# AuroraEchos/Sound-Event-Localization-and-Detection

Measured on AMD Instinct MI355X. Metric: train-step samples/sec (8ch x 128mel x 512T), higher is better.
Workload: dtype f32; 1 GPU; c3: DQSELD-TCN-S1-PHI_8ch train step, F=128 T=512 (U=L=192, SURVEY F3), batch 32/GPU, random-init weights; global_batch=32, parallelism=dp1, step_mode=graph (auto: probe 9.50 ms recorded / 10.73 ms eager per step), deterministic=True

## Files before the change

include/seld_hip.h:

```cpp
#ifndef SELD_HIP_H
#define SELD_HIP_H

#include <stddef.h>
#include <stdint.h>

#ifdef __cplusplus
extern "C" {
#endif

#define SELD_OK            0
#define SELD_EINVAL       -1
#define SELD_EWORKSPACE   -2
#define SELD_ELAUNCH      -3
#define SELD_EUNSUPPORTED -4

int         seld_abi_version(void);
const char* seld_build_arch(void);
int         seld_last_hip_error(void);
int         seld_env_reload(void);
int         seld_tuning_build(void);

typedef struct seld_conv_desc {
    int32_t algebra;
    int32_t ndim;
    int32_t N, Cin, Cout;
    int32_t in[2];
    int32_t k[2];
    int32_t stride[2];
    int32_t pad[2];
    int32_t dil[2];
    int32_t groups;
} seld_conv_desc;

#define SELD_EPI_NONE        0
// ... 210 lines not shown

int seld_bn_act_fwd(const float* x, int32_t N, int32_t C, int32_t S, const float* mean, const float* invstd,
                    const float* gamma, const float* beta, int32_t act, float* y, void* stream);

int seld_bn_act_bwd_reduce(const float* dy, const float* x, const float* y, int32_t N, int32_t C, int32_t S,
                           const float* mean, const float* invstd, const float* gamma, const float* beta,
                           int32_t act, float* dgamma_dbeta , void* stream);
int seld_bn_act_bwd_apply(const float* dy, const float* x, const float* y, int32_t N, int32_t C, int32_t S,
                          const float* mean, const float* invstd, const float* gamma, const float* beta,
                          int32_t act, const float* dgamma_dbeta, int32_t train, float* dx, void* stream);

int seld_bn_act_bwd_fused(const float* dy, const float* x, const float* y, int32_t N, int32_t C, int32_t S,
                          const float* mean, const float* invstd, const float* gamma, int32_t act,
                          float* dgamma_dbeta, const float* dy2, float* dx, void* stream);

int seld_gate_fwd(const float* yf, const float* yg, int32_t N, int32_t C, int32_t S,
                  const float* mean_f, const float* invstd_f, const float* gamma_f, const float* beta_f,
                  const float* mean_g, const float* invstd_g, const float* gamma_g, const float* beta_g,
                  const float* mask, float* y, void* stream);
int seld_gate_bwd_reduce(const float* dy, const float* yf, const float* yg, int32_t N, int32_t C, int32_t S,
                         const float* mean_f, const float* invstd_f, const float* gamma_f, const float* beta_f,
                         const float* mean_g, const float* invstd_g, const float* gamma_g, const float* beta_g,
                         const float* mask, float* red, void* stream);
int seld_gate_bwd_apply(const float* dy, const float* yf, const float* yg, int32_t N, int32_t C, int32_t S,
                        const float* mean_f, const float* invstd_f, const float* gamma_f, const float* beta_f,
                        const float* mean_g, const float* invstd_g, const float* gamma_g, const float* beta_g,
                        const float* mask, const float* red, int32_t train, float* dyf, float* dyg, void* stream);

int seld_hcq_first_pool(const seld_conv_desc* desc, const float* x, const float* wpack, const float* bias,
                        const float* gamma, int32_t want_stats, float* y, float* stats, float* pool_raw, uint8_t* idx,
// ... 10 lines not shown
size_t seld_first_stage_bwd_workspace(const seld_conv_desc* desc);
int seld_first_stage_bwd(const seld_conv_desc* desc, const float* x, const float* dout, const float* out, const float* raw,
                         const uint8_t* idx, const float* mean, const float* invstd, const float* gamma, const float* beta,
                         const float* bias, const double* gram, const float* wg, float* dgamma, float* dbeta,
                         float* const dw[8], float drop_p, void* workspace, size_t workspace_bytes, void* stream);

int seld_bn_pool_finish(const float* raw, int32_t N, int32_t C, int32_t S , const float* mean,
                        const float* invstd, const float* gamma, const float* beta, float* pooled, float p, uint64_t seed,
                        uint64_t offset, const uint64_t* state, float* out, void* stream);

int seld_gate_bwd_fused(const float* dy, const float* yf, const float* yg, int32_t N, int32_t C, int32_t S,
                        const float* mean_f, const float* invstd_f, const float* gamma_f, const float* beta_f,
                        const float* mean_g, const float* invstd_g, const float* gamma_g, const float* beta_g,
                        const float* mask, float* red, float* dyf, float* dyg, void* stream);

size_t seld_hcq_pack_floats(const seld_conv_desc* desc, int32_t mode, int32_t npair);
int seld_hcq_pack(const seld_conv_desc* desc, int32_t mode, int32_t npair, const float* const wA[8],
                  const float* const wB[8], float* wpack, void* stream);
int seld_hcq_conv(const seld_conv_desc* desc, int32_t mode, int32_t npair, const float* x, const float* x2,
                  const float* wpack, float* const y[2], const float* const bias[2], const int32_t epilogue[2],
                  const float* const addend[2], float* const stats[2], void* stream);
int seld_hcq_kernel_label(const seld_conv_desc* desc, int32_t mode, int32_t npair, char* buf, int32_t buflen);
size_t seld_hcq_pack_entry_bytes(void);
int seld_hcq_pack_entry(const seld_conv_desc* desc, int32_t mode, int32_t npair, const float* const wA[8],
                        const float* const wB[8], float* wpack, void* entry_host);
int seld_hcq_pack_table(const void* table_dev, int32_t nentries, int64_t max_floats, void* stream);
int seld_hcq_pack_flat(const void* table_dev, const int32_t* starts_dev, int32_t nentries, int32_t total_blocks,
                       void* stream);

int seld_hcq_wgrad_supported(const seld_conv_desc* desc, int32_t npair);
// ... 132 lines not shown
```

sound-event-localization-and-detection_amd/csrc/abi.hip:

```cpp
#include <mutex>
#include <stdio.h>
#include <stdlib.h>
#include "common.h"
#include "env.h"

namespace seld {
thread_local int g_last_hip_error = 0;

static SeldEnv g_env;
static bool g_env_loaded = false;
static std::mutex g_env_mutex;

static bool flag(const char* name) { const char* e = getenv(name); return e && *e; }
static long long bounded(const char* name, long long lo, long long hi, long long dflt) {
    const char* e = getenv(name);
    if (!e || !*e) return dflt;
    char* end = nullptr;
    const long long v = strtoll(e, &end, 10);
    return (end == e || v < lo || v > hi) ? dflt : v;
}

static void load_env_locked() {
    SeldEnv e;
    if (const char* c = getenv("SELD_CONV_CFG")) {
// ... 3 lines not shown
    e.conv_novec = flag("SELD_CONV_NOVEC");
    e.conv_nofast = flag("SELD_CONV_NOFAST");
    e.conv_no_smallk = flag("SELD_CONV_NO_SMALLK");
    e.no_fwd_pair = flag("SELD_NO_FWD_PAIR");
    e.conv_pair = flag("SELD_CONV_PAIR");
    e.conv_no_hcq = flag("SELD_CONV_NO_HCQ");
    e.hcq_wgrad_dq = flag("SELD_HCQ_WGRAD_DQ");
    e.stft_radix2 = flag("SELD_STFT_RADIX2");
    e.hcq_no_first = flag("SELD_HCQ_NO_FIRST");
    e.hcq_no_pool = flag("SELD_HCQ_NO_POOL");
    e.hcq_wgrad_row = flag("SELD_HCQ_WGRAD_ROW");
    e.deterministic = flag("SELD_DETERMINISTIC");
    e.wgrad_norow = flag("SELD_WGRAD_NOROW");
    e.wgrad_slow = flag("SELD_WGRAD_SLOW");
    e.mha_no_mfma = flag("SELD_MHA_NO_MFMA");
    e.wgrad_cfg = (int)bounded("SELD_WGRAD_CFG", 0, 5, -1);
    e.wgrad_wgs = bounded("SELD_WGRAD_WGS", 1, 1 << 20, 0);
    e.smallk_wgs = bounded("SELD_SMALLK_WGS", 1, 1 << 20, 0);
#ifdef SELD_TUNING
    e.vec_dbg = (int)bounded("SELD_VEC_DBG", 0, 63, 0);
    e.wgrad_dbg = (int)bounded("SELD_WGRAD_DBG", 0, 3, 0);
    e.smallk_dbg = (int)bounded("SELD_SMALLK_DBG", 0, 1023, 0);
    e.smallk_nw = bounded("SELD_SMALLK_NW", 4, 8, 4) == 8 ? 8 : 4;
#endif
    g_env = e;
    g_env_loaded = true;
}

const SeldEnv& env() {
    if (!g_env_loaded) {
// ... 5 lines not shown
}

extern "C" int seld_env_reload(void) {
    std::lock_guard<std::mutex> lk(seld::g_env_mutex);
    seld::load_env_locked();
    return SELD_OK;
}
extern "C" int seld_tuning_build(void) {
#ifdef SELD_TUNING
    return 1;
#else
    return 0;
#endif
}

extern "C" int seld_abi_version(void) { return 2; }
extern "C" const char* seld_build_arch(void) { return "gfx950"; }
extern "C" int seld_last_hip_error(void) { return seld::g_last_hip_error; }
```

sound-event-localization-and-detection_amd/csrc/env.h:

```cpp
#pragma once

namespace seld {

struct SeldEnv {
    int conv_cfg_ct = 0, conv_cfg_pt = 0;
    bool conv_novec = false, conv_nofast = false, conv_no_smallk = false, no_fwd_pair = false, conv_pair = false;
    bool hcq_wgrad_dq = false;
    bool conv_no_hcq = false;
    bool hcq_wgrad_row = false;
    bool hcq_no_pool = false;
    bool stft_radix2 = false;
    bool hcq_no_first = false;
    bool deterministic = false;
    bool wgrad_norow = false, wgrad_slow = false, mha_no_mfma = false;
    int wgrad_cfg = -1;
    long long wgrad_wgs = 0, smallk_wgs = 0;
    int vec_dbg = 0, wgrad_dbg = 0, smallk_dbg = 0, smallk_nw = 4;
};

const SeldEnv& env();

}
```

sound-event-localization-and-detection_amd/csrc/nn_ops.hip:

```cpp
#include "common.h"
#include "env.h"

namespace seld {

__device__ __forceinline__ float act_apply(float z, int act) {
    switch (act) {
        case SELD_ACT_RELU: return z > 0.f ? z : 0.f;
        case SELD_ACT_TANH: return tanhf(z);
        case SELD_ACT_SIGMOID: return 1.0f / (1.0f + expf(-z));
        default: return z;
    }
}
__device__ __forceinline__ float act_grad_from_y(float y, int act) {
    switch (act) {
        case SELD_ACT_RELU: return y > 0.f ? 1.f : 0.f;
        case SELD_ACT_TANH: return 1.f - y * y;
        case SELD_ACT_SIGMOID: return y * (1.f - y);
        default: return 1.f;
    }
}

constexpr int RED_CHUNK = 8192;

template <typename F>
// ... 384 lines not shown
            for (int e = 0; e < 4; ++e) {
                const float t = gate_tanh(ff[e] * af + bf);
                const float sg = gate_sig(gg[e] * ag + bg);
                const float d = dd[e] * mk;
                const float dzf = d * sg * (1.f - t * t);
                const float dzg = d * t * sg * (1.f - sg);
                of[e] = af * (dzf - kf1 - (ff[e] - muf) * isf * kf2);
                og[e] = ag * (dzg - kg1 - (gg[e] - mug) * isg * kg2);
            }
            *reinterpret_cast<float4*>(dyf + base + s) = make_float4(of[0], of[1], of[2], of[3]);
            *reinterpret_cast<float4*>(dyg + base + s) = make_float4(og[0], og[1], og[2], og[3]);
        }
    }
}

constexpr int CH_THREADS = 512;

template <int NV>
__device__ __forceinline__ void channel_block_sum(float (&v)[NV]) {
    __shared__ float part[NV][CH_THREADS / 64];
    const int wave = threadIdx.x >> 6, lane = threadIdx.x & 63;
#pragma unroll
    for (int k = 0; k < NV; ++k) {
        const float s = wave_sum(v[k]);
        if (lane == 0) part[k][wave] = s;
    }
    __syncthreads();
#pragma unroll
    for (int k = 0; k < NV; ++k) {
        float t = 0.f;
#pragma unroll
        for (int w = 0; w < CH_THREADS / 64; ++w) t += part[k][w];
        v[k] = t;
    }
}

__device__ __forceinline__ float4 ld4(const float* p) { return *reinterpret_cast<const float4*>(p); }

template <int PER>
__global__ __launch_bounds__(CH_THREADS) void bn_act_bwd_channel_kernel(
    const float* __restrict__ dy, const float* __restrict__ x, const float* __restrict__ y, int N, int C, int S,
    const float* __restrict__ mean, const float* __restrict__ invstd, const float* __restrict__ gamma, int act,
    float* __restrict__ red, const float* __restrict__ dy2, float* __restrict__ dx, float inv_count) {
    const int c = blockIdx.x;
    const int S4 = S >> 2, G = N * S4;
    const float mu = mean[c], is = invstd[c], a = gamma[c] * is;
    float4 dz[PER], xh[PER];
    float v[2] = {0.f, 0.f};
    float4 ds_[PER], xs_[PER], ys_[PER];
#pragma unroll
    for (int k = 0; k < PER; ++k) {
        const int g = min((int)threadIdx.x + k * CH_THREADS, G - 1);
        const int n = g / S4, s4 = g - n * S4;
        const size_t o = ((size_t)n * C + c) * S + (size_t)s4 * 4;
        ds_[k] = ld4(dy + o); xs_[k] = ld4(x + o); ys_[k] = ld4(y + o);
        if (dy2) {
            const float4 e = ld4(dy2 + o);
            ds_[k].x += e.x; ds_[k].y += e.y; ds_[k].z += e.z; ds_[k].w += e.w;
        }
    }
    __builtin_amdgcn_sched_barrier(0);
// ... 24 lines not shown
        const int g = (int)threadIdx.x + k * CH_THREADS;
        if (g < G) {
            const int n = g / S4, s4 = g - n * S4;
            const size_t o = ((size_t)n * C + c) * S + (size_t)s4 * 4;
            float4 r = make_float4(a * (dz[k].x - k1 - xh[k].x * k2), a * (dz[k].y - k1 - xh[k].y * k2),
                                   a * (dz[k].z - k1 - xh[k].z * k2), a * (dz[k].w - k1 - xh[k].w * k2));
            *reinterpret_cast<float4*>(dx + o) = r;
        }
    }
}

template <int PER>
__global__ __launch_bounds__(CH_THREADS) void gate_bwd_channel_kernel(
    const float* __restrict__ dy, const float* __restrict__ yf, const float* __restrict__ yg, int N, int C, int S,
    GateBN bn, const float* __restrict__ mask, float* __restrict__ red, float* __restrict__ dyf,
    float* __restrict__ dyg, float inv_count) {
    const int c = blockIdx.x;
    const int S4 = S >> 2, G = N * S4;
    const float muf = bn.mean_f[c], isf = bn.invstd_f[c], af = bn.gamma_f[c] * isf, bf = bn.beta_f[c] - muf * af;
    const float mug = bn.mean_g[c], isg = bn.invstd_g[c], ag = bn.gamma_g[c] * isg, bg = bn.beta_g[c] - mug * ag;
    float dzf[PER][4], dzg[PER][4], fh[PER][4], gh[PER][4];
    float v[4] = {0.f, 0.f, 0.f, 0.f};
    float4 d4s[PER], f4s[PER], g4s[PER];
    float mks[PER];
#pragma unroll
    for (int k = 0; k < PER; ++k) {
        const int g = min((int)threadIdx.x + k * CH_THREADS, G - 1);
        const int n = g / S4, s4 = g - n * S4;
        const size_t o = ((size_t)n * C + c) * S + (size_t)s4 * 4;
        d4s[k] = ld4(dy + o); f4s[k] = ld4(yf + o); g4s[k] = ld4(yg + o);
        mks[k] = mask ? mask[n * C + c] : 1.0f;
    }
    __builtin_amdgcn_sched_barrier(0);
#pragma unroll
    for (int k = 0; k < PER; ++k) {
// ... 370 lines not shown
    return check_launch();
}

extern "C" int seld_bn_act_bwd_apply(const float* dy, const float* x, const float* y, int32_t N, int32_t C, int32_t S,
                                     const float* mean, const float* invstd, const float* gamma, const float* beta,
                                     int32_t act, const float* red, int32_t train, float* dx, void* stream) {
    (void)beta;
    if (!dy || !x || !y || !dx || (train && !red)) return SELD_EINVAL;
    const long long total = (long long)N * C * S;
    const float inv_count = 1.0f / (float)((long long)N * S);
    hipLaunchKernelGGL(bn_act_bwd_apply_kernel, dim3(grid_for(total / 4 + 1)), dim3(256), 0, ST(stream), dy, x, y, total,
                       C, S, mean, invstd, gamma, act, red, inv_count, train, dx);
    return check_launch();
}

extern "C" int seld_bn_act_bwd_fused(const float* dy, const float* x, const float* y, int32_t N, int32_t C, int32_t S,
                                     const float* mean, const float* invstd, const float* gamma, int32_t act,
                                     float* red, const float* dy2, float* dx, void* stream) {
    if (!dy || !x || !y || !red || !mean || !invstd || !gamma || N <= 0 || C <= 0 || S <= 0) return SELD_EINVAL;
    const long long G = (long long)N * S / 4;
    if ((S & 3) || G > 16LL * CH_THREADS) return SELD_EUNSUPPORTED;
    const float inv_count = 1.0f / (float)((long long)N * S);
    const int per = (int)((G + CH_THREADS - 1) / CH_THREADS);
#define SELD_BN_CH(P)                                                                                                   \
    hipLaunchKernelGGL(bn_act_bwd_channel_kernel<P>, dim3(C), dim3(CH_THREADS), 0, ST(stream), dy, x, y, N, C, S, mean,  \
                       invstd, gamma, act, red, dy2, dx, inv_count)
    if (per <= 1) SELD_BN_CH(1);
    else if (per <= 2) SELD_BN_CH(2);
    else if (per <= 4) SELD_BN_CH(4);
    else if (per <= 8) SELD_BN_CH(8);
    else SELD_BN_CH(16);
#undef SELD_BN_CH
    return check_launch();
}

static GateBN mk_gate(const float* mean_f, const float* invstd_f, const float* gamma_f, const float* beta_f,
                      const float* mean_g, const float* invstd_g, const float* gamma_g, const float* beta_g) {
    GateBN b{mean_f, invstd_f, gamma_f, beta_f, mean_g, invstd_g, gamma_g, beta_g};
    return b;
}

extern "C" int seld_gate_fwd(const float* yf, const float* yg, int32_t N, int32_t C, int32_t S, const float* mean_f,
                             const float* invstd_f, const float* gamma_f, const float* beta_f, const float* mean_g,
                             const float* invstd_g, const float* gamma_g, const float* beta_g, const float* mask,
                             float* y, void* stream) {
    if (!yf || !yg || !y) return SELD_EINVAL;
    const long long total = (long long)N * C * S;
    if (S % 4 == 0 && (long long)N * C < (1LL << 31))
// ... 28 lines not shown
                                   void* stream) {
    if (!dy || !yf || !yg || !dyf || !dyg || (train && !red)) return SELD_EINVAL;
    const long long total = (long long)N * C * S;
    const float inv_count = 1.0f / (float)((long long)N * S);
    if (S % 4 == 0 && (long long)N * C < (1LL << 31))
        hipLaunchKernelGGL(gate_bwd_apply_row_kernel, dim3(row_grid((long long)N * C)), dim3(256), 0, ST(stream), dy, yf, yg,
                           N * C, C, S, mk_gate(mean_f, invstd_f, gamma_f, beta_f, mean_g, invstd_g, gamma_g, beta_g), mask, red,
                           inv_count, train, dyf, dyg);
    else
        hipLaunchKernelGGL(gate_bwd_apply_kernel, dim3(grid_for(total / 4 + 1)), dim3(256), 0, ST(stream), dy, yf, yg, total,
                           C, S, mk_gate(mean_f, invstd_f, gamma_f, beta_f, mean_g, invstd_g, gamma_g, beta_g), mask, red,
                           inv_count, train, dyf, dyg);
    return check_launch();
}

extern "C" int seld_gate_bwd_fused(const float* dy, const float* yf, const float* yg, int32_t N, int32_t C, int32_t S,
                                   const float* mean_f, const float* invstd_f, const float* gamma_f, const float* beta_f,
                                   const float* mean_g, const float* invstd_g, const float* gamma_g, const float* beta_g,
                                   const float* mask, float* red, float* dyf, float* dyg, void* stream) {
    if (!dy || !yf || !yg || !red || !dyf || !dyg || N <= 0 || C <= 0 || S <= 0) return SELD_EINVAL;
    const long long G = (long long)N * S / 4;
    if ((S & 3) || G > 8LL * CH_THREADS) return SELD_EUNSUPPORTED;
    const float inv_count = 1.0f / (float)((long long)N * S);
    const int per = (int)((G + CH_THREADS - 1) / CH_THREADS);
    const GateBN bn = mk_gate(mean_f, invstd_f, gamma_f, beta_f, mean_g, invstd_g, gamma_g, beta_g);
#define SELD_GATE_CH(P)                                                                                                 \
    hipLaunchKernelGGL(gate_bwd_channel_kernel<P>, dim3(C), dim3(CH_THREADS), 0, ST(stream), dy, yf, yg, N, C, S, bn,    \
                       mask, red, dyf, dyg, inv_count)
    if (per <= 1) SELD_GATE_CH(1);
    else if (per <= 2) SELD_GATE_CH(2);
    else if (per <= 4) SELD_GATE_CH(4);
    else SELD_GATE_CH(8);
#undef SELD_GATE_CH
    return check_launch();
}

extern "C" int seld_act_fwd(const float* x, int64_t n, int32_t act, float* y, void* stream) {
    if (!x || !y || n < 0) return SELD_EINVAL;
    if (n == 0) return SELD_OK;
    hipLaunchKernelGGL(act_fwd_kernel, dim3(grid_for(n)), dim3(256), 0, ST(stream), x, (long long)n, act, y);
    return check_launch();
}
extern "C" int seld_act_bwd(const float* dy, const float* y, int64_t n, int32_t act, float* dx, void* stream) {
    if (!dy || !y || !dx || n < 0) return SELD_EINVAL;
    if (n == 0) return SELD_OK;
    hipLaunchKernelGGL(act_bwd_kernel, dim3(grid_for(n)), dim3(256), 0, ST(stream), dy, y, (long long)n, act, dx);
    return check_launch();
}
// ... 104 lines not shown
```

sound-event-localization-and-detection_amd/hip_ops/norm_act.py:

```python
import os

import torch

from .. import _lib as L
from ._core import _req


def _ncs(x):
    N, C = x.shape[0], x.shape[1]
    S = 1
    for d in x.shape[2:]:
        S *= d
    return N, C, S


STATS_REPLICAS = 64


_stats_pool = {}


def new_stats(C, device):
    free = _stats_pool.get((C, device, torch.cuda.current_stream(device).cuda_stream))
    if free:
        return free.pop()
    t = torch.zeros(STATS_REPLICAS * 2 * C, device=device, dtype=torch.float32)
    t._seld_pooled = True
    return t


def channel_stats(x, out=None):
    N, C, S = _ncs(x)
    stats = out if out is not None else new_stats(C, x.device)
    L.check(L.lib().seld_channel_stats(L.ptr(x), N, C, S, L.ptr(stats), L.current_stream()), "seld_channel_stats")
    return stats


def bn_prepare(x, running_mean, running_var, training, momentum, eps, stats=None, num_batches_tracked=None):
    N, C, S = _ncs(x)
    mean = torch.empty(C, device=x.device, dtype=torch.float32)
    invstd = torch.empty(C, device=x.device, dtype=torch.float32)
    if training:
        if stats is None:
# ... 84 lines not shown
    w._seld_base_param = param
    return w


def axpy_(dst_first, src, n):
    L.check(L.lib().seld_accumulate(L.ptr(dst_first), L.ptr(src), n, L.current_stream()), "seld_accumulate")


def _one_pass_ok(N, S, limit):
    return S % 4 == 0 and N * S <= limit and not os.environ.get("SELD_BN_TWO_PASS")


class BnActFn(torch.autograd.Function):

    @staticmethod
    def forward(ctx, x, gamma, beta, running_mean, running_var, training, momentum, eps, act, stats, nbt, twin):
        x = _req(x, "x")
        N, C, S = _ncs(x)
        mean, invstd = bn_prepare(x, running_mean, running_var, training, momentum, eps, stats, nbt)
        y = torch.empty_like(x)
        L.check(L.lib().seld_bn_act_fwd(L.ptr(x), N, C, S, L.ptr(mean), L.ptr(invstd), L.ptr(gamma), L.ptr(beta),
                                        act, L.ptr(y), L.current_stream()), "seld_bn_act_fwd")
        ctx.training, ctx.act = training, act
        ctx.bn_params = (gamma, beta)
        ctx.save_for_backward(x, y, mean, invstd)
        ctx.twin = twin
        if twin:
            ctx.set_materialize_grads(False)
            return y, y.view_as(y)
        return y

    @staticmethod
    def backward(ctx, dy, dy2=None):
        x, y, mean, invstd = ctx.saved_tensors
        gamma, beta = ctx.bn_params
        if dy is None:
            dy, dy2 = dy2, None
        if dy is None:
            return (None,) * 12
        dy = _req(dy, "dy")
        dy2 = _req(dy2, "dy2") if dy2 is not None else None
        none = (None,) * 9
        N, C, S = _ncs(x)
        slot, clean = _claim_grad_slots((gamma, beta))
        st = L.current_stream()
        if ctx.training and _one_pass_ok(N, S, 32768):
            red = slot if slot is not None else torch.zeros(2 * C, device=x.device, dtype=torch.float32)
            dx = torch.empty_like(x) if ctx.needs_input_grad[0] else None
            L.check(L.lib().seld_bn_act_bwd_fused(L.ptr(dy), L.ptr(x), L.ptr(y), N, C, S, L.ptr(mean), L.ptr(invstd),
                                                  L.ptr(gamma), ctx.act, L.ptr(red), L.ptr(dy2), L.ptr(dx), st),
                    "seld_bn_act_bwd_fused")
            if slot is not None:
                return (dx, None, None) + none
            return (dx, red[:C], red[C:]) + none
        if dy2 is not None:
            dy = dy + dy2
        red = slot if clean else torch.zeros(2 * C, device=x.device, dtype=torch.float32)
        L.check(L.lib().seld_bn_act_bwd_reduce(L.ptr(dy), L.ptr(x), L.ptr(y), N, C, S, L.ptr(mean), L.ptr(invstd),
                                               L.ptr(gamma), L.ptr(beta), ctx.act, L.ptr(red), st),
                "seld_bn_act_bwd_reduce")
        dx = None
        if ctx.needs_input_grad[0]:
            dx = torch.empty_like(x)
            L.check(L.lib().seld_bn_act_bwd_apply(L.ptr(dy), L.ptr(x), L.ptr(y), N, C, S, L.ptr(mean), L.ptr(invstd),
                                                  L.ptr(gamma), L.ptr(beta), ctx.act, L.ptr(red), int(ctx.training),
                                                  L.ptr(dx), st), "seld_bn_act_bwd_apply")
        if slot is not None:
            if not clean:
                axpy_(slot, red, 2 * C)
            return (dx, None, None) + none
        return (dx, red[:C], red[C:]) + none


def bn_act(x, bn, act, stats=None, twin=False):
    return BnActFn.apply(x, bn.weight, bn.bias, bn.running_mean, bn.running_var, bn.training,
                         bn.momentum if bn.momentum is not None else 0.1, bn.eps, act, stats, _nbt(bn), twin)


class GateFn(torch.autograd.Function):

    @staticmethod
    def forward(ctx, yf, yg, gf, bf, rmf, rvf, gg, bg, rmg, rvg, training, momentum, eps, mask, nbt_f, nbt_g,
                stats_f=None, stats_g=None):
        yf, yg = _req(yf, "yf"), _req(yg, "yg")
        N, C, S = _ncs(yf)
        if (training and stats_f is not None and stats_g is not None and getattr(stats_f, "_seld_pooled", False)
                and getattr(stats_g, "_seld_pooled", False)):
            mf, isf, mg, isg = (torch.empty(C, device=yf.device, dtype=torch.float32) for _ in range(4))
            L.check(L.lib().seld_bn_finalize2_ex(L.ptr(stats_f), L.ptr(stats_g), C, N * S, eps, momentum, L.ptr(mf),
                                                 L.ptr(isf), L.ptr(rmf), L.ptr(rvf), L.ptr(nbt_f), L.ptr(mg),
                                                 L.ptr(isg), L.ptr(rmg), L.ptr(rvg), L.ptr(nbt_g), 1,
                                                 L.current_stream()), "seld_bn_finalize2_ex")
            key = (C, yf.device, torch.cuda.current_stream(yf.device).cuda_stream)
            _stats_pool.setdefault(key, []).extend((stats_f, stats_g))
        else:
            mf, isf = bn_prepare(yf, rmf, rvf, training, momentum, eps, stats_f, nbt_f)
            mg, isg = bn_prepare(yg, rmg, rvg, training, momentum, eps, stats_g, nbt_g)
        y = torch.empty_like(yf)
        L.check(L.lib().seld_gate_fwd(L.ptr(yf), L.ptr(yg), N, C, S, L.ptr(mf), L.ptr(isf), L.ptr(gf), L.ptr(bf),
                                      L.ptr(mg), L.ptr(isg), L.ptr(gg), L.ptr(bg), L.ptr(mask), L.ptr(y),
                                      L.current_stream()), "seld_gate_fwd")
        ctx.training = training
        ctx.has_mask = mask is not None
        ctx.bn_params = (gf, bf, gg, bg)
        ctx.save_for_backward(yf, yg, mf, isf, mg, isg, *([mask] if mask is not None else []))
        return y

    @staticmethod
    def backward(ctx, dy):
        yf, yg, mf, isf, mg, isg, *rest = ctx.saved_tensors
        gf, bf, gg, bg = ctx.bn_params
        mask = rest[0] if ctx.has_mask else None
        dy = _req(dy, "dy")
        N, C, S = _ncs(yf)
        slot, clean = _claim_grad_slots((gf, bf, gg, bg))
        st = L.current_stream()
        if ctx.training and _one_pass_ok(N, S, 16384):
            red = slot if slot is not None else torch.zeros(4 * C, device=yf.device, dtype=torch.float32)
            dyf, dyg = torch.empty_like(yf), torch.empty_like(yg)
            L.check(L.lib().seld_gate_bwd_fused(L.ptr(dy), L.ptr(yf), L.ptr(yg), N, C, S, L.ptr(mf), L.ptr(isf),
                                                L.ptr(gf), L.ptr(bf), L.ptr(mg), L.ptr(isg), L.ptr(gg), L.ptr(bg),
                                                L.ptr(mask), L.ptr(red), L.ptr(dyf), L.ptr(dyg), st),
                    "seld_gate_bwd_fused")
            if slot is not None:
                return (dyf, dyg) + (None,) * 16
            return (dyf, dyg, red[:C], red[C:2 * C], None, None, red[2 * C:3 * C], red[3 * C:], None, None,
                    None, None, None, None, None, None, None, None)
        red = slot if clean else torch.zeros(4 * C, device=yf.device, dtype=torch.float32)
        args = (L.ptr(dy), L.ptr(yf), L.ptr(yg), N, C, S, L.ptr(mf), L.ptr(isf), L.ptr(gf), L.ptr(bf),
                L.ptr(mg), L.ptr(isg), L.ptr(gg), L.ptr(bg), L.ptr(mask))
        L.check(L.lib().seld_gate_bwd_reduce(*args, L.ptr(red), st), "seld_gate_bwd_reduce")
        dyf, dyg = torch.empty_like(yf), torch.empty_like(yg)
        L.check(L.lib().seld_gate_bwd_apply(*args, L.ptr(red), int(ctx.training), L.ptr(dyf), L.ptr(dyg), st),
                "seld_gate_bwd_apply")
        if slot is not None:
            if not clean:
                axpy_(slot, red, 4 * C)
            return (dyf, dyg) + (None,) * 16
        return (dyf, dyg, red[:C], red[C:2 * C], None, None, red[2 * C:3 * C], red[3 * C:], None, None,
                None, None, None, None, None, None, None, None)


def gate(yf, yg, bn_f, bn_g, mask=None, stats_f=None, stats_g=None):
    return GateFn.apply(yf, yg, bn_f.weight, bn_f.bias, bn_f.running_mean, bn_f.running_var,
                        bn_g.weight, bn_g.bias, bn_g.running_mean, bn_g.running_var, bn_f.training,
                        bn_f.momentum if bn_f.momentum is not None else 0.1, bn_f.eps, mask, _nbt(bn_f), _nbt(bn_g),
                        stats_f, stats_g)


class ActFn(torch.autograd.Function):
    @staticmethod
    def forward(ctx, x, act):
        x = _req(x, "x")
        y = torch.empty_like(x)
        L.check(L.lib().seld_act_fwd(L.ptr(x), x.numel(), act, L.ptr(y), L.current_stream()), "seld_act_fwd")
        ctx.act = act
        ctx.save_for_backward(y)
        return y

    @staticmethod
    def backward(ctx, dy):
        (y,) = ctx.saved_tensors
# ... 159 lines not shown

def transpose12(x):
    return TransposeFn.apply(x)


_identity_cache = {}


def gate_plain(yf, yg, mask=None):
    C = yf.shape[1]
    key = (yf.device, C)
    if key not in _identity_cache:
        _identity_cache[key] = (torch.zeros(C, device=yf.device), torch.ones(C, device=yf.device))
    zero, one = _identity_cache[key]

    return GateFn.apply(yf, yg, one, zero, zero, one, one, zero, zero, one, False, 0.1, 0.0, mask, None, None, None, None)
```

Measured before the change: 3658 samples/s.

## Fuse BN stat finalization into act/gate forward and clear pooled stats in backward

Adds forward kernels that reduce the replicated BN partial stats, compute mean/invstd, update the running stats, and apply the BN+activation or gate all in one launch. The separate finalize kernel is dropped for small shapes. The backward fused kernels now also zero the lent stats buffers, so no separate clear or memset is needed before reuse. This cuts kernel launches and small-op overhead per layer in exchange for redundant per-block stat reduction and more complex lifetime tracking of pooled stat buffers.

New measurement: 3689 samples/s (median of 6 runs). About the same (+0.9%).

```diff
diff --git a/include/seld_hip.h b/include/seld_hip.h
--- a/include/seld_hip.h
+++ b/include/seld_hip.h
@@ -18,6 +18,7 @@
 const char* seld_build_arch(void);
 int         seld_last_hip_error(void);
 int         seld_env_reload(void);
+int         seld_fused_small(void);
 int         seld_tuning_build(void);
 
 typedef struct seld_conv_desc {
@@ -258,6 +259,14 @@
                           const float* mean, const float* invstd, const float* gamma, int32_t act,
                           float* dgamma_dbeta, const float* dy2, float* dx, void* stream);
 
+int seld_bn_act_bwd_fused_clear(const float* dy, const float* x, const float* y, int32_t N, int32_t C, int32_t S,
+                                const float* mean, const float* invstd, const float* gamma, int32_t act,
+                                float* dgamma_dbeta, const float* dy2, float* dx, float* clear_stats, void* stream);
+
+int seld_bn_act_fwd_stats(const float* x, int32_t N, int32_t C, int32_t S, const float* stats, float eps, float momentum,
+                          const float* gamma, const float* beta, int32_t act, float* mean, float* invstd,
+                          float* running_mean, float* running_var, int64_t* num_batches_tracked, float* y, void* stream);
+
 int seld_gate_fwd(const float* yf, const float* yg, int32_t N, int32_t C, int32_t S,
                   const float* mean_f, const float* invstd_f, const float* gamma_f, const float* beta_f,
                   const float* mean_g, const float* invstd_g, const float* gamma_g, const float* beta_g,
@@ -298,6 +307,17 @@
                         const float* mean_g, const float* invstd_g, const float* gamma_g, const float* beta_g,
                         const float* mask, float* red, float* dyf, float* dyg, void* stream);
 
+int seld_gate_bwd_fused_clear(const float* dy, const float* yf, const float* yg, int32_t N, int32_t C, int32_t S,
+                              const float* mean_f, const float* invstd_f, const float* gamma_f, const float* beta_f,
+                              const float* mean_g, const float* invstd_g, const float* gamma_g, const float* beta_g,
+                              const float* mask, float* red, float* dyf, float* dyg, float* clear_f, float* clear_g,
+                              void* stream);
+int seld_gate_fwd_stats(const float* yf, const float* yg, int32_t N, int32_t C, int32_t S, const float* stats_f,
+                        const float* stats_g, float eps, float momentum, const float* gamma_f, const float* beta_f,
+                        const float* gamma_g, const float* beta_g, float* mean_f, float* invstd_f, float* running_mean_f,
+                        float* running_var_f, int64_t* nbt_f, float* mean_g, float* invstd_g, float* running_mean_g,
+                        float* running_var_g, int64_t* nbt_g, const float* mask, float* y, void* stream);
+
 size_t seld_hcq_pack_floats(const seld_conv_desc* desc, int32_t mode, int32_t npair);
 int seld_hcq_pack(const seld_conv_desc* desc, int32_t mode, int32_t npair, const float* const wA[8],
                   const float* const wB[8], float* wpack, void* stream);
diff --git a/sound-event-localization-and-detection_amd/csrc/abi.hip b/sound-event-localization-and-detection_amd/csrc/abi.hip
--- a/sound-event-localization-and-detection_amd/csrc/abi.hip
+++ b/sound-event-localization-and-detection_amd/csrc/abi.hip
@@ -41,6 +41,7 @@
     e.wgrad_norow = flag("SELD_WGRAD_NOROW");
     e.wgrad_slow = flag("SELD_WGRAD_SLOW");
     e.mha_no_mfma = flag("SELD_MHA_NO_MFMA");
+    if (const char* c = getenv("SELD_FUSED_SMALL")) e.fused_small = !(c[0] == '0' && c[1] == 0);
     e.wgrad_cfg = (int)bounded("SELD_WGRAD_CFG", 0, 5, -1);
     e.wgrad_wgs = bounded("SELD_WGRAD_WGS", 1, 1 << 20, 0);
     e.smallk_wgs = bounded("SELD_SMALLK_WGS", 1, 1 << 20, 0);
@@ -76,6 +77,8 @@
 #endif
 }
 
+extern "C" int seld_fused_small(void) { return seld::env().fused_small ? 1 : 0; }
+
 extern "C" int seld_abi_version(void) { return 2; }
 extern "C" const char* seld_build_arch(void) { return "gfx950"; }
 extern "C" int seld_last_hip_error(void) { return seld::g_last_hip_error; }
diff --git a/sound-event-localization-and-detection_amd/csrc/env.h b/sound-event-localization-and-detection_amd/csrc/env.h
--- a/sound-event-localization-and-detection_amd/csrc/env.h
+++ b/sound-event-localization-and-detection_amd/csrc/env.h
@@ -13,6 +13,7 @@
     bool hcq_no_first = false;
     bool deterministic = false;
     bool wgrad_norow = false, wgrad_slow = false, mha_no_mfma = false;
+    bool fused_small = true;
     int wgrad_cfg = -1;
     long long wgrad_wgs = 0, smallk_wgs = 0;
     int vec_dbg = 0, wgrad_dbg = 0, smallk_dbg = 0, smallk_nw = 4;
diff --git a/sound-event-localization-and-detection_amd/csrc/nn_ops.hip b/sound-event-localization-and-detection_amd/csrc/nn_ops.hip
--- a/sound-event-localization-and-detection_amd/csrc/nn_ops.hip
+++ b/sound-event-localization-and-detection_amd/csrc/nn_ops.hip
@@ -422,6 +422,101 @@
     }
 }
 
+struct BnStats {
+    const float* stats; float* mean; float* invstd; float* rmean; float* rvar; long long* nbt;
+};
+
+__device__ __forceinline__ void bn_finalize_wave(const BnStats& f, int C, int c, double count, float eps, float momentum,
+                                                 bool publish, float* __restrict__ out2) {
+    static_assert(SELD_STATS_REPLICAS == 64, "one lane per replica row");
+    const int lane = threadIdx.x & 63;
+    const float* p1 = f.stats + (size_t)lane * 2 * C + c;
+    double s1 = (double)p1[0], s2 = (double)p1[C];
+#pragma unroll
+    for (int o = 32; o > 0; o >>= 1) {
+        s1 += __shfl_xor(s1, o, 64);
+        s2 += __shfl_xor(s2, o, 64);
+    }
+    if (lane != 0) return;
+    const double m = s1 / count;
+    double var = s2 / count - m * m;
+    if (var < 0.0) var = 0.0;
+    const float mf = (float)m, is = (float)(1.0 / sqrt(var + (double)eps));
+    out2[0] = mf;
+    out2[1] = is;
+    if (!publish) return;
+    if (c == 0 && f.nbt) *f.nbt += 1;
+    f.mean[c] = mf;
+    f.invstd[c] = is;
+    if (f.rmean) f.rmean[c] = (1.f - momentum) * f.rmean[c] + momentum * (float)m;
+    if (f.rvar) {
+        const double unbiased = count > 1.0 ? var * count / (count - 1.0) : var;
+        f.rvar[c] = (1.f - momentum) * f.rvar[c] + momentum * (float)unbiased;
+    }
+}
+
+__global__ __launch_bounds__(256) void bn_act_fwd_stats_kernel(const float* __restrict__ x, int N, int C, int S, int rpw,
+                                                               BnStats st, double count, float eps, float momentum,
+                                                               const float* __restrict__ gamma, const float* __restrict__ beta,
+                                                               int act, float* __restrict__ y) {
+    __shared__ float cst[2];
+    const int wave = __builtin_amdgcn_readfirstlane((int)threadIdx.x >> 6), lane = threadIdx.x & 63;
+    const int c = blockIdx.x;
+    if (wave == 0) bn_finalize_wave(st, C, c, count, eps, momentum, blockIdx.y == 0, cst);
+    __syncthreads();
+    const float a = gamma[c] * cst[1];
+    const float b = beta[c] - cst[0] * a;
+    const int n_end = min(N, ((int)blockIdx.y + 1) * rpw);
+    for (int n = blockIdx.y * rpw + wave; n < n_end; n += 4) {
+        const size_t base = ((size_t)n * C + c) * S;
+        for (int s = lane * 4; s < S; s += 256) {
+            float4 v = *reinterpret_cast<const float4*>(x + base + s);
+            v.x = act_apply(v.x * a + b, act);
+            v.y = act_apply(v.y * a + b, act);
+            v.z = act_apply(v.z * a + b, act);
+            v.w = act_apply(v.w * a + b, act);
+            *reinterpret_cast<float4*>(y + base + s) = v;
+        }
+    }
+}
+
+__global__ __launch_bounds__(256) void gate_fwd_stats_kernel(const float* __restrict__ yf, const float* __restrict__ yg,
+                                                             int N, int C, int S, int rpw, BnStats sf, BnStats sg,
+                                                             double count, float eps, float momentum,
+                                                             const float* __restrict__ gamma_f, const float* __restrict__ beta_f,
+                                                             const float* __restrict__ gamma_g, const float* __restrict__ beta_g,
+                                                             const float* __restrict__ mask, float* __restrict__ y) {
+    __shared__ float cst[4];
+    const int wave = __builtin_amdgcn_readfirstlane((int)threadIdx.x >> 6), lane = threadIdx.x & 63;
+    const int c = blockIdx.x;
+    if (wave == 0) bn_finalize_wave(sf, C, c, count, eps, momentum, blockIdx.y == 0, cst);
+    else if (wave == 1) bn_finalize_wave(sg, C, c, count, eps, momentum, blockIdx.y == 0, cst + 2);
+    __syncthreads();
+    const float af = gamma_f[c] * cst[1], bf = beta_f[c] - cst[0] * af;
+    const float ag = gamma_g[c] * cst[3], bg = beta_g[c] - cst[2] * ag;
+    const int n_end = min(N, ((int)blockIdx.y + 1) * rpw);
+    for (int n = blockIdx.y * rpw + wave; n < n_end; n += 4) {
+        const int row = n * C + c;
+        const float mk = mask ? mask[row] : 1.0f;
+        const size_t base = (size_t)row * S;
+        for (int s = lane * 4; s < S; s += 256) {
+            const float4 f = *reinterpret_cast<const float4*>(yf + base + s);
+            const float4 g = *reinterpret_cast<const float4*>(yg + base + s);
+            float4 o;
+            o.x = gate_tanh(f.x * af + bf) * gate_sig(g.x * ag + bg) * mk;
+            o.y = gate_tanh(f.y * af + bf) * gate_sig(g.y * ag + bg) * mk;
+            o.z = gate_tanh(f.z * af + bf) * gate_sig(g.z * ag + bg) * mk;
+            o.w = gate_tanh(f.w * af + bf) * gate_sig(g.w * ag + bg) * mk;
+            *reinterpret_cast<float4*>(y + base + s) = o;
+        }
+    }
+}
+
+__device__ __forceinline__ void clear_channel_stats(float* __restrict__ stats, int C, int c) {
+    if (stats && threadIdx.x < 2 * SELD_STATS_REPLICAS)
+        stats[(size_t)(threadIdx.x >> 1) * 2 * C + (threadIdx.x & 1) * C + c] = 0.f;
+}
+
 constexpr int CH_THREADS = 512;
 
 template <int NV>
@@ -449,10 +544,12 @@
 __global__ __launch_bounds__(CH_THREADS) void bn_act_bwd_channel_kernel(
     const float* __restrict__ dy, const float* __restrict__ x, const float* __restrict__ y, int N, int C, int S,
     const float* __restrict__ mean, const float* __restrict__ invstd, const float* __restrict__ gamma, int act,
-    float* __restrict__ red, const float* __restrict__ dy2, float* __restrict__ dx, float inv_count) {
+    float* __restrict__ red, const float* __restrict__ dy2, float* __restrict__ dx, float inv_count,
+    float* __restrict__ clear) {
     const int c = blockIdx.x;
     const int S4 = S >> 2, G = N * S4;
     const float mu = mean[c], is = invstd[c], a = gamma[c] * is;
+    clear_channel_stats(clear, C, c);
     float4 dz[PER], xh[PER];
     float v[2] = {0.f, 0.f};
     float4 ds_[PER], xs_[PER], ys_[PER];
@@ -507,11 +604,13 @@
 __global__ __launch_bounds__(CH_THREADS) void gate_bwd_channel_kernel(
     const float* __restrict__ dy, const float* __restrict__ yf, const float* __restrict__ yg, int N, int C, int S,
     GateBN bn, const float* __restrict__ mask, float* __restrict__ red, float* __restrict__ dyf,
-    float* __restrict__ dyg, float inv_count) {
+    float* __restrict__ dyg, float inv_count, float* __restrict__ clear_f, float* __restrict__ clear_g) {
     const int c = blockIdx.x;
     const int S4 = S >> 2, G = N * S4;
     const float muf = bn.mean_f[c], isf = bn.invstd_f[c], af = bn.gamma_f[c] * isf, bf = bn.beta_f[c] - muf * af;
     const float mug = bn.mean_g[c], isg = bn.invstd_g[c], ag = bn.gamma_g[c] * isg, bg = bn.beta_g[c] - mug * ag;
+    clear_channel_stats(clear_f, C, c);
+    clear_channel_stats(clear_g, C, c);
     float dzf[PER][4], dzg[PER][4], fh[PER][4], gh[PER][4];
     float v[4] = {0.f, 0.f, 0.f, 0.f};
     float4 d4s[PER], f4s[PER], g4s[PER];
@@ -912,9 +1011,9 @@
     return check_launch();
 }
 
-extern "C" int seld_bn_act_bwd_fused(const float* dy, const float* x, const float* y, int32_t N, int32_t C, int32_t S,
-                                     const float* mean, const float* invstd, const float* gamma, int32_t act,
-                                     float* red, const float* dy2, float* dx, void* stream) {
+extern "C" int seld_bn_act_bwd_fused_clear(const float* dy, const float* x, const float* y, int32_t N, int32_t C, int32_t S,
+                                           const float* mean, const float* invstd, const float* gamma, int32_t act,
+                                           float* red, const float* dy2, float* dx, float* clear_stats, void* stream) {
     if (!dy || !x || !y || !red || !mean || !invstd || !gamma || N <= 0 || C <= 0 || S <= 0) return SELD_EINVAL;
     const long long G = (long long)N * S / 4;
     if ((S & 3) || G > 16LL * CH_THREADS) return SELD_EUNSUPPORTED;
@@ -922,7 +1021,7 @@
     const int per = (int)((G + CH_THREADS - 1) / CH_THREADS);
 #define SELD_BN_CH(P)                                                                                                   \
     hipLaunchKernelGGL(bn_act_bwd_channel_kernel<P>, dim3(C), dim3(CH_THREADS), 0, ST(stream), dy, x, y, N, C, S, mean,  \
-                       invstd, gamma, act, red, dy2, dx, inv_count)
+                       invstd, gamma, act, red, dy2, dx, inv_count, clear_stats)
     if (per <= 1) SELD_BN_CH(1);
     else if (per <= 2) SELD_BN_CH(2);
     else if (per <= 4) SELD_BN_CH(4);
@@ -930,6 +1029,12 @@
     else SELD_BN_CH(16);
 #undef SELD_BN_CH
     return check_launch();
+}
+
+extern "C" int seld_bn_act_bwd_fused(const float* dy, const float* x, const float* y, int32_t N, int32_t C, int32_t S,
+                                     const float* mean, const float* invstd, const float* gamma, int32_t act,
+                                     float* red, const float* dy2, float* dx, void* stream) {
+    return seld_bn_act_bwd_fused_clear(dy, x, y, N, C, S, mean, invstd, gamma, act, red, dy2, dx, nullptr, stream);
 }
 
 static GateBN mk_gate(const float* mean_f, const float* invstd_f, const float* gamma_f, const float* beta_f,
@@ -988,10 +1093,11 @@
     return check_launch();
 }
 
-extern "C" int seld_gate_bwd_fused(const float* dy, const float* yf, const float* yg, int32_t N, int32_t C, int32_t S,
-                                   const float* mean_f, const float* invstd_f, const float* gamma_f, const float* beta_f,
-                                   const float* mean_g, const float* invstd_g, const float* gamma_g, const float* beta_g,
-                                   const float* mask, float* red, float* dyf, float* dyg, void* stream) {
+extern "C" int seld_gate_bwd_fused_clear(const float* dy, const float* yf, const float* yg, int32_t N, int32_t C, int32_t S,
+                                         const float* mean_f, const float* invstd_f, const float* gamma_f, const float* beta_f,
+                                         const float* mean_g, const float* invstd_g, const float* gamma_g, const float* beta_g,
+                                         const float* mask, float* red, float* dyf, float* dyg, float* clear_f,
+                                         float* clear_g, void* stream) {
     if (!dy || !yf || !yg || !red || !dyf || !dyg || N <= 0 || C <= 0 || S <= 0) return SELD_EINVAL;
     const long long G = (long long)N * S / 4;
     if ((S & 3) || G > 8LL * CH_THREADS) return SELD_EUNSUPPORTED;
@@ -1000,12 +1106,56 @@
     const GateBN bn = mk_gate(mean_f, invstd_f, gamma_f, beta_f, mean_g, invstd_g, gamma_g, beta_g);
 #define SELD_GATE_CH(P)                                                                                                 \
     hipLaunchKernelGGL(gate_bwd_channel_kernel<P>, dim3(C), dim3(CH_THREADS), 0, ST(stream), dy, yf, yg, N, C, S, bn,    \
-                       mask, red, dyf, dyg, inv_count)
+                       mask, red, dyf, dyg, inv_count, clear_f, clear_g)
     if (per <= 1) SELD_GATE_CH(1);
     else if (per <= 2) SELD_GATE_CH(2);
     else if (per <= 4) SELD_GATE_CH(4);
     else SELD_GATE_CH(8);
 #undef SELD_GATE_CH
+    return check_launch();
+}
+extern "C" int seld_gate_bwd_fused(const float* dy, const float* yf, const float* yg, int32_t N, int32_t C, int32_t S,
+                                   const float* mean_f, const float* invstd_f, const float* gamma_f, const float* beta_f,
+                                   const float* mean_g, const float* invstd_g, const float* gamma_g, const float* beta_g,
+                                   const float* mask, float* red, float* dyf, float* dyg, void* stream) {
+    return seld_gate_bwd_fused_clear(dy, yf, yg, N, C, S, mean_f, invstd_f, gamma_f, beta_f, mean_g, invstd_g, gamma_g,
+                                     beta_g, mask, red, dyf, dyg, nullptr, nullptr, stream);
+}
+
+static inline int rows_per_wg(int N, int C) {
+    int rpw = 16;
+    while (rpw > 4 && (long long)C * ((N + rpw - 1) / rpw) < 768) rpw >>= 1;
+    return rpw;
+}
+extern "C" int seld_bn_act_fwd_stats(const float* x, int32_t N, int32_t C, int32_t S, const float* stats, float eps,
+                                     float momentum, const float* gamma, const float* beta, int32_t act, float* mean,
+                                     float* invstd, float* running_mean, float* running_var, int64_t* num_batches_tracked,
+                                     float* y, void* stream) {
+    if (!x || !y || !stats || !mean || !invstd || !gamma || !beta || N <= 0 || C <= 0 || S <= 0) return SELD_EINVAL;
+    if ((S & 3) || C > 65535) return SELD_EUNSUPPORTED;
+    const int rpw = rows_per_wg(N, C);
+    if ((N + rpw - 1) / rpw > 65535) return SELD_EUNSUPPORTED;
+    const BnStats st{stats, mean, invstd, running_mean, running_var, (long long*)num_batches_tracked};
+    hipLaunchKernelGGL(bn_act_fwd_stats_kernel, dim3(C, (N + rpw - 1) / rpw), dim3(256), 0, ST(stream), x, N, C, S, rpw, st,
+                       (double)((long long)N * S), eps, momentum, gamma, beta, act, y);
+    return check_launch();
+}
+extern "C" int seld_gate_fwd_stats(const float* yf, const float* yg, int32_t N, int32_t C, int32_t S, const float* stats_f,
+                                   const float* stats_g, float eps, float momentum, const float* gamma_f,
+                                   const float* beta_f, const float* gamma_g, const float* beta_g, float* mean_f,
+                                   float* invstd_f, float* running_mean_f, float* running_var_f, int64_t* nbt_f,
+                                   float* mean_g, float* invstd_g, float* running_mean_g, float* running_var_g,
+                                   int64_t* nbt_g, const float* mask, float* y, void* stream) {
+    if (!yf || !yg || !y || !stats_f || !stats_g || !mean_f || !invstd_f || !mean_g || !invstd_g || !gamma_f || !beta_f ||
+        !gamma_g || !beta_g || N <= 0 || C <= 0 || S <= 0)
+        return SELD_EINVAL;
+    if ((S & 3) || C > 65535 || (long long)N * C >= (1LL << 31)) return SELD_EUNSUPPORTED;
+    const int rpw = rows_per_wg(N, C);
+    if ((N + rpw - 1) / rpw > 65535) return SELD_EUNSUPPORTED;
+    const BnStats sf{stats_f, mean_f, invstd_f, running_mean_f, running_var_f, (long long*)nbt_f};
+    const BnStats sg{stats_g, mean_g, invstd_g, running_mean_g, running_var_g, (long long*)nbt_g};
+    hipLaunchKernelGGL(gate_fwd_stats_kernel, dim3(C, (N + rpw - 1) / rpw), dim3(256), 0, ST(stream), yf, yg, N, C, S, rpw,
+                       sf, sg, (double)((long long)N * S), eps, momentum, gamma_f, beta_f, gamma_g, beta_g, mask, y);
     return check_launch();
 }
 
diff --git a/sound-event-localization-and-detection_amd/hip_ops/norm_act.py b/sound-event-localization-and-detection_amd/hip_ops/norm_act.py
--- a/sound-event-localization-and-detection_amd/hip_ops/norm_act.py
+++ b/sound-event-localization-and-detection_amd/hip_ops/norm_act.py
@@ -21,12 +21,39 @@
 
 
 def new_stats(C, device):
-    free = _stats_pool.get((C, device, torch.cuda.current_stream(device).cuda_stream))
+    key = (C, device, torch.cuda.current_stream(device).cuda_stream)
+    free = _stats_pool.get(key)
     if free:
         return free.pop()
+    if torch.cuda.is_current_stream_capturing() and fused_small():
+        for other, bufs in _stats_pool.items():
+            if other[:2] == key[:2] and bufs:
+                return bufs.pop()
     t = torch.zeros(STATS_REPLICAS * 2 * C, device=device, dtype=torch.float32)
     t._seld_pooled = True
     return t
+
+
+def fused_small():
+    return bool(L.lib().seld_fused_small())
+
+
+def _stream_key(C, device):
+    return (C, device, torch.cuda.current_stream(device).cuda_stream)
+
+
+def _lend_stats(ctx, *stats):
+    ctx.lent_stats = stats
+    ctx.lent_key = _stream_key(stats[0].numel() // (2 * STATS_REPLICAS), stats[0].device)
+
+
+def _return_stats(ctx, zeroed):
+    stats, ctx.lent_stats = getattr(ctx, "lent_stats", None), None
+    if stats:
+        if not zeroed:
+            for t in stats:
+                t.zero_()
+        _stats_pool.setdefault(ctx.lent_key, []).extend(stats)
 
 
 def channel_stats(x, out=None):
@@ -141,13 +168,27 @@
 class BnActFn(torch.autograd.Function):
 
     @staticmethod
-    def forward(ctx, x, gamma, beta, running_mean, running_var, training, momentum, eps, act, stats, nbt, twin):
+    def forward(ctx, x, gamma, beta, running_mean, running_var, training, momentum, eps, act, stats, nbt, twin,
+                fuse=False):
         x = _req(x, "x")
         N, C, S = _ncs(x)
-        mean, invstd = bn_prepare(x, running_mean, running_var, training, momentum, eps, stats, nbt)
         y = torch.empty_like(x)
-        L.check(L.lib().seld_bn_act_fwd(L.ptr(x), N, C, S, L.ptr(mean), L.ptr(invstd), L.ptr(gamma), L.ptr(beta),
-                                        act, L.ptr(y), L.current_stream()), "seld_bn_act_fwd")
+        ctx.lent_stats = None
+        fuse = fuse and training and _one_pass_ok(N, S, 32768) and fused_small()
+        if fuse and stats is None:
+            stats = channel_stats(x)
+        if fuse and getattr(stats, "_seld_pooled", False):
+            mean = torch.empty(C, device=x.device, dtype=torch.float32)
+            invstd = torch.empty(C, device=x.device, dtype=torch.float32)
+            L.check(L.lib().seld_bn_act_fwd_stats(L.ptr(x), N, C, S, L.ptr(stats), eps, momentum, L.ptr(gamma), L.ptr(beta),
+                                                  act, L.ptr(mean), L.ptr(invstd), L.ptr(running_mean),
+                                                  L.ptr(running_var), L.ptr(nbt), L.ptr(y), L.current_stream()),
+                    "seld_bn_act_fwd_stats")
+            _lend_stats(ctx, stats)
+        else:
+            mean, invstd = bn_prepare(x, running_mean, running_var, training, momentum, eps, stats, nbt)
+            L.check(L.lib().seld_bn_act_fwd(L.ptr(x), N, C, S, L.ptr(mean), L.ptr(invstd), L.ptr(gamma), L.ptr(beta),
+                                            act, L.ptr(y), L.current_stream()), "seld_bn_act_fwd")
         ctx.training, ctx.act = training, act
         ctx.bn_params = (gamma, beta)
         ctx.save_for_backward(x, y, mean, invstd)
@@ -164,22 +205,26 @@
         if dy is None:
             dy, dy2 = dy2, None
         if dy is None:
-            return (None,) * 12
+            _return_stats(ctx, zeroed=False)
+            return (None,) * 13
         dy = _req(dy, "dy")
         dy2 = _req(dy2, "dy2") if dy2 is not None else None
-        none = (None,) * 9
+        none = (None,) * 10
         N, C, S = _ncs(x)
         slot, clean = _claim_grad_slots((gamma, beta))
         st = L.current_stream()
         if ctx.training and _one_pass_ok(N, S, 32768):
             red = slot if slot is not None else torch.zeros(2 * C, device=x.device, dtype=torch.float32)
             dx = torch.empty_like(x) if ctx.needs_input_grad[0] else None
-            L.check(L.lib().seld_bn_act_bwd_fused(L.ptr(dy), L.ptr(x), L.ptr(y), N, C, S, L.ptr(mean), L.ptr(invstd),
-                                                  L.ptr(gamma), ctx.act, L.ptr(red), L.ptr(dy2), L.ptr(dx), st),
-                    "seld_bn_act_bwd_fused")
+            lent = ctx.lent_stats[0] if ctx.lent_stats else None
+            L.check(L.lib().seld_bn_act_bwd_fused_clear(L.ptr(dy), L.ptr(x), L.ptr(y), N, C, S, L.ptr(mean),
+                                                        L.ptr(invstd), L.ptr(gamma), ctx.act, L.ptr(red), L.ptr(dy2),
+                                                        L.ptr(dx), L.ptr(lent), st), "seld_bn_act_bwd_fused_clear")
+            _return_stats(ctx, zeroed=True)
             if slot is not None:
                 return (dx, None, None) + none
             return (dx, red[:C], red[C:]) + none
+        _return_stats(ctx, zeroed=False)
         if dy2 is not None:
             dy = dy + dy2
         red = slot if clean else torch.zeros(2 * C, device=x.device, dtype=torch.float32)
@@ -200,17 +245,35 @@
 
 
 def bn_act(x, bn, act, stats=None, twin=False):
+    fuse = torch.is_grad_enabled() and any(t.requires_grad for t in (x, bn.weight, bn.bias))
     return BnActFn.apply(x, bn.weight, bn.bias, bn.running_mean, bn.running_var, bn.training,
-                         bn.momentum if bn.momentum is not None else 0.1, bn.eps, act, stats, _nbt(bn), twin)
+                         bn.momentum if bn.momentum is not None else 0.1, bn.eps, act, stats, _nbt(bn), twin, fuse)
 
 
 class GateFn(torch.autograd.Function):
 
     @staticmethod
     def forward(ctx, yf, yg, gf, bf, rmf, rvf, gg, bg, rmg, rvg, training, momentum, eps, mask, nbt_f, nbt_g,
-                stats_f=None, stats_g=None):
+                stats_f=None, stats_g=None, fuse=False):
         yf, yg = _req(yf, "yf"), _req(yg, "yg")
         N, C, S = _ncs(yf)
+        y = torch.empty_like(yf)
+        ctx.lent_stats = None
+        both_pooled = (training and stats_f is not None and stats_g is not None and getattr(stats_f, "_seld_pooled", False)
+                       and getattr(stats_g, "_seld_pooled", False))
+        if fuse and both_pooled and _one_pass_ok(N, S, 16384) and fused_small():
+            mf, isf, mg, isg = (torch.empty(C, device=yf.device, dtype=torch.float32) for _ in range(4))
+            L.check(L.lib().seld_gate_fwd_stats(L.ptr(yf), L.ptr(yg), N, C, S, L.ptr(stats_f), L.ptr(stats_g), eps, momentum,
+                                                L.ptr(gf), L.ptr(bf), L.ptr(gg), L.ptr(bg), L.ptr(mf), L.ptr(isf),
+                                                L.ptr(rmf), L.ptr(rvf), L.ptr(nbt_f), L.ptr(mg), L.ptr(isg), L.ptr(rmg),
+                                                L.ptr(rvg), L.ptr(nbt_g), L.ptr(mask), L.ptr(y), L.current_stream()),
+                    "seld_gate_fwd_stats")
+            _lend_stats(ctx, stats_f, stats_g)
+            ctx.training = training
+            ctx.has_mask = mask is not None
+            ctx.bn_params = (gf, bf, gg, bg)
+            ctx.save_for_backward(yf, yg, mf, isf, mg, isg, *([mask] if mask is not None else []))
+            return y
         if (training and stats_f is not None and stats_g is not None and getattr(stats_f, "_seld_pooled", False)
                 and getattr(stats_g, "_seld_pooled", False)):
             mf, isf, mg, isg = (torch.empty(C, device=yf.device, dtype=torch.float32) for _ in range(4))
@@ -223,7 +286,6 @@
         else:
             mf, isf = bn_prepare(yf, rmf, rvf, training, momentum, eps, stats_f, nbt_f)
             mg, isg = bn_prepare(yg, rmg, rvg, training, momentum, eps, stats_g, nbt_g)
-        y = torch.empty_like(yf)
         L.check(L.lib().seld_gate_fwd(L.ptr(yf), L.ptr(yg), N, C, S, L.ptr(mf), L.ptr(isf), L.ptr(gf), L.ptr(bf),
                                       L.ptr(mg), L.ptr(isg), L.ptr(gg), L.ptr(bg), L.ptr(mask), L.ptr(y),
                                       L.current_stream()), "seld_gate_fwd")
@@ -245,14 +307,17 @@
         if ctx.training and _one_pass_ok(N, S, 16384):
             red = slot if slot is not None else torch.zeros(4 * C, device=yf.device, dtype=torch.float32)
             dyf, dyg = torch.empty_like(yf), torch.empty_like(yg)
-            L.check(L.lib().seld_gate_bwd_fused(L.ptr(dy), L.ptr(yf), L.ptr(yg), N, C, S, L.ptr(mf), L.ptr(isf),
-                                                L.ptr(gf), L.ptr(bf), L.ptr(mg), L.ptr(isg), L.ptr(gg), L.ptr(bg),
-                                                L.ptr(mask), L.ptr(red), L.ptr(dyf), L.ptr(dyg), st),
-                    "seld_gate_bwd_fused")
+            lent_f, lent_g = ctx.lent_stats if ctx.lent_stats else (None, None)
+            L.check(L.lib().seld_gate_bwd_fused_clear(L.ptr(dy), L.ptr(yf), L.ptr(yg), N, C, S, L.ptr(mf), L.ptr(isf),
+                                                      L.ptr(gf), L.ptr(bf), L.ptr(mg), L.ptr(isg), L.ptr(gg), L.ptr(bg),
+                                                      L.ptr(mask), L.ptr(red), L.ptr(dyf), L.ptr(dyg), L.ptr(lent_f),
+                                                      L.ptr(lent_g), st), "seld_gate_bwd_fused_clear")
+            _return_stats(ctx, zeroed=True)
             if slot is not None:
-                return (dyf, dyg) + (None,) * 16
+                return (dyf, dyg) + (None,) * 17
             return (dyf, dyg, red[:C], red[C:2 * C], None, None, red[2 * C:3 * C], red[3 * C:], None, None,
-                    None, None, None, None, None, None, None, None)
+                    None, None, None, None, None, None, None, None, None)
+        _return_stats(ctx, zeroed=False)
         red = slot if clean else torch.zeros(4 * C, device=yf.device, dtype=torch.float32)
         args = (L.ptr(dy), L.ptr(yf), L.ptr(yg), N, C, S, L.ptr(mf), L.ptr(isf), L.ptr(gf), L.ptr(bf),
                 L.ptr(mg), L.ptr(isg), L.ptr(gg), L.ptr(bg), L.ptr(mask))
@@ -263,16 +328,17 @@
         if slot is not None:
             if not clean:
                 axpy_(slot, red, 4 * C)
-            return (dyf, dyg) + (None,) * 16
+            return (dyf, dyg) + (None,) * 17
         return (dyf, dyg, red[:C], red[C:2 * C], None, None, red[2 * C:3 * C], red[3 * C:], None, None,
-                None, None, None, None, None, None, None, None)
+                None, None, None, None, None, None, None, None, None)
 
 
 def gate(yf, yg, bn_f, bn_g, mask=None, stats_f=None, stats_g=None):
+    fuse = torch.is_grad_enabled() and any(t.requires_grad for t in (yf, yg, bn_f.weight, bn_f.bias, bn_g.weight, bn_g.bias))
     return GateFn.apply(yf, yg, bn_f.weight, bn_f.bias, bn_f.running_mean, bn_f.running_var,
                         bn_g.weight, bn_g.bias, bn_g.running_mean, bn_g.running_var, bn_f.training,
                         bn_f.momentum if bn_f.momentum is not None else 0.1, bn_f.eps, mask, _nbt(bn_f), _nbt(bn_g),
-                        stats_f, stats_g)
+                        stats_f, stats_g, fuse)
 
 
 class ActFn(torch.autograd.Function):
@@ -462,4 +528,4 @@
         _identity_cache[key] = (torch.zeros(C, device=yf.device), torch.ones(C, device=yf.device))
     zero, one = _identity_cache[key]
 
-    return GateFn.apply(yf, yg, one, zero, zero, one, one, zero, zero, one, False, 0.1, 0.0, mask, None, None, None, None)
+    return GateFn.apply(yf, yg, one, zero, zero, one, one, zero, zero, one, False, 0.1, 0.0, mask, None, None, None, None, False)
```
